# robertteleng/aria-slam

Measured on AMD Instinct MI355X. Metric: frames/s ORB extract+BF-match, 640x480 @2000 kp, higher is better.
Workload: dtype u8

## Files before the change

### aria_slam_amd/csrc/orb_kernels.hip

```cpp
#include <hip/hip_runtime.h>

#include <cfloat>
#include <cstdint>
#include <cstdlib>

#include "common.h"
#include "orb_device.h"
#include "orb_kernels.h"

namespace aria {

struct PatternLaneMajor { uint32_t w[16][16]; };
constexpr PatternLaneMajor make_pattern_lane_major() {
    constexpr int src[1024] = {
#include "orb_pattern_31.inc"
    };
    PatternLaneMajor p{};
    for (int l = 0; l < 16; l++)
        for (int it = 0; it < 16; it++) {
            const int t = 16 * it + l;
            p.w[l][it] = ((uint32_t)(src[4 * t] & 0xFF)) | ((uint32_t)(src[4 * t + 1] & 0xFF) << 8) |
                         ((uint32_t)(src[4 * t + 2] & 0xFF) << 16) | ((uint32_t)(src[4 * t + 3] & 0xFF) << 24);
        }
    return p;
}
__device__ __attribute__((aligned(16))) const PatternLaneMajor kPattern31 = make_pattern_lane_major();

#define ARIA_UMAX_LIST {15, 15, 15, 15, 14, 14, 14, 13, 13, 12, 11, 10, 9, 8, 6, 3}

struct IcMaskLaneMajor { uint32_t m[16][16]; };
constexpr IcMaskLaneMajor make_ic_mask() {
    constexpr int umax[16] = ARIA_UMAX_LIST;
    IcMaskLaneMajor t{};
    for (int l = 0; l < 16; l++)
        for (int k = 0; k < 16; k++) {
            const int r = 2 * k + (l >> 3), j = l & 7;
            uint32_t w = 0;
            for (int b = 0; b < 4 && r < 31; b++) {
                const int u = 4 * j + b - 15, v = r - 15;
                const int au = u < 0 ? -u : u, av = v < 0 ? -v : v;
                if (au <= 15 && au <= umax[av]) w |= 0xFFu << (8 * b);
            }
            t.m[l][k] = w;
        }
    return t;
}
__device__ __attribute__((aligned(16))) const IcMaskLaneMajor kIcMask = make_ic_mask();

typedef short s2v __attribute__((ext_vector_type(2)));
__device__ __forceinline__ void harris_row_pairs(const uint8_t* rowp, int xs, int sh, bool dword_ok, uint32_t* E) {
    uint32_t w0, w1, w2;
    if (dword_ok) {
        const uint32_t* q = reinterpret_cast<const uint32_t*>(rowp + xs);
        w0 = q[0]; w1 = q[1]; w2 = q[2];
    } else {
        const uint8_t* q = rowp + xs;
        w0 = (uint32_t)q[0] | ((uint32_t)q[1] << 8) | ((uint32_t)q[2] << 16) | ((uint32_t)q[3] << 24);
        w1 = (uint32_t)q[4] | ((uint32_t)q[5] << 8) | ((uint32_t)q[6] << 16) | ((uint32_t)q[7] << 24);
        w2 = (uint32_t)q[8] | ((uint32_t)q[9] << 8) | ((uint32_t)q[10] << 16) | ((uint32_t)q[11] << 24);
    }
    const uint32_t a = __builtin_amdgcn_alignbyte(w1, w0, (uint32_t)sh);
    const uint32_t b = __builtin_amdgcn_alignbyte(w2, w1, (uint32_t)sh);
    E[0] = __builtin_amdgcn_perm(0u, a, 0x0c010c00u);
    E[1] = __builtin_amdgcn_perm(0u, a, 0x0c030c02u);
    E[2] = __builtin_amdgcn_perm(0u, b, 0x0c010c00u);
    E[3] = __builtin_amdgcn_perm(0u, b, 0x0c030c02u);
    E[4] = (w2 >> (8 * sh)) & 0xFFu;
}

__device__ __forceinline__ uint32_t pk16_add(uint32_t a, uint32_t b) {
    return __builtin_bit_cast(uint32_t, __builtin_bit_cast(s2v, a) + __builtin_bit_cast(s2v, b));
}
__device__ __forceinline__ uint32_t pk16_sub(uint32_t a, uint32_t b) {
    return __builtin_bit_cast(uint32_t, __builtin_bit_cast(s2v, a) - __builtin_bit_cast(s2v, b));
}

__device__ __forceinline__ float harris_response(const uint8_t* img, int pitch, int x, int y, bool dword_ok) {
    int a = 0, b = 0, c = 0;
    const int xs = (x - 4) & ~3, sh = (x - 4) & 3;
    const uint8_t* base = img + (int64_t)(y - 4) * pitch;
    uint32_t R[9][5];
#pragma unroll
    for (int r = 0; r < 9; r++) harris_row_pairs(base + (int64_t)r * pitch, xs, sh, dword_ok, R[r]);
#pragma unroll
    for (int i = 1; i <= 7; i++) {
        uint32_t sE[5], dE[5];
#pragma unroll
        for (int k = 0; k < 5; k++) {
            sE[k] = pk16_add(pk16_add(R[i - 1][k], R[i + 1][k]), pk16_add(R[i][k], R[i][k]));
            dE[k] = pk16_sub(R[i + 1][k], R[i - 1][k]);
        }
#pragma unroll
        for (int k = 0; k < 4; k++) {
            uint32_t ix = pk16_sub(sE[k + 1], sE[k]);
            const uint32_t dO = __builtin_amdgcn_alignbit(dE[k + 1], dE[k], 16);
            uint32_t iy = pk16_add(pk16_add(dE[k], dE[k + 1]), pk16_add(dO, dO));
            if (k == 3) { ix &= 0xFFFFu; iy &= 0xFFFFu; }
            const s2v vx = __builtin_bit_cast(s2v, ix), vy = __builtin_bit_cast(s2v, iy);
            a = __builtin_amdgcn_sdot2(vx, vx, a, false);
            b = __builtin_amdgcn_sdot2(vy, vy, b, false);
            c = __builtin_amdgcn_sdot2(vx, vy, c, false);
        }
    }
    const float scale = 1.f / ((1 << 2) * 7 * 255.f);
    const float scale_sq_sq = scale * scale * scale * scale;
    const float k = 0.04f;
    return ((float)a * (float)b - (float)c * (float)c - k * ((float)a + (float)b) * ((float)a + (float)b)) * scale_sq_sq;
}

__device__ void select_ovf_item(const Plan& P, const FrameSrc& S, const uint8_t* __restrict__ raw,
                                const uint32_t* __restrict__ cand, const int* __restrict__ cand_cnt,
                                uint4* __restrict__ sel, int* __restrict__ sel_cnt, int* __restrict__ err,
                                int* __restrict__ ovf, unsigned long long* __restrict__ keys, long long keys_cap,
                                uint4* __restrict__ osel, int osel_cap, int frame, int l, int* s_hist, int* s_misc);

template <bool INLINE_OVF, int NT>
__global__ __launch_bounds__(NT) void k_select(Plan P, FrameSrc S, const uint8_t* __restrict__ raw,
                                                const uint32_t* __restrict__ cand, const int* __restrict__ cand_cnt,
                                                uint4* __restrict__ sel, int* __restrict__ sel_cnt,
                                                int* __restrict__ err, unsigned long long* __restrict__ stamps,
                                                int* __restrict__ ovf, int2* __restrict__ ovf_items,
                                                unsigned long long* __restrict__ ovf_keys, long long ovf_keys_cap,
                                                uint4* __restrict__ osel, int osel_cap, int force_bitonic) {
    static_assert(kLevels == 8, "level rotation below assumes 8 levels");
    const int l = (int)((blockIdx.x + blockIdx.y) & 7u), frame = blockIdx.y;
#define SSTAMP(k) do { if (stamps && threadIdx.x == 0) stamps[((size_t)blockIdx.y * kLevels + l) * 8 + (k)] = __builtin_amdgcn_s_memtime(); } while (0)
    SSTAMP(0);
    extern __shared__ __attribute__((aligned(16))) unsigned long long s_keys[];
    __shared__ int s_hist[256];
    __shared__ int s_misc[4];
    __shared__ int s_wsum[NT / 64];
    __shared__ int s_bin[1024];

    const int tid = threadIdx.x;
    const bool lead = tid < 256;
    const LevelGeom g = P.lv[l];
    const uint32_t* clist = cand + (int64_t)frame * P.cand_frame_entries + g.cand_off;
    const int n = min(cand_cnt[frame * kLevels + l], g.cand_cap);
    const int q = g.quota;
    const int kSortCap = P.sort_cap;

    if (q == 0 || n == 0) {
        if (tid == 0) sel_cnt[frame * kLevels + l] = 0;
        return;
    }
    if (lead) s_hist[tid] = 0;
    if (tid == 0) { s_misc[1] = 0; s_misc[2] = 0; }
    __syncthreads();
    constexpr int kUnroll = 8;
    for (int i0 = 0; i0 < n; i0 += NT * kUnroll) {
        uint32_t v[kUnroll];
#pragma unroll
        for (int u = 0; u < kUnroll; u++) {
            const int i = i0 + u * NT + tid;
            v[u] = i < n ? clist[i] : 0u;
        }
#pragma unroll
        for (int u = 0; u < kUnroll; u++)
            if (i0 + u * NT + tid < n) atomicAdd(&s_hist[v[u] >> 22], 1);
    }
    __syncthreads();
    SSTAMP(1);
    {
        const int lane = tid & 63, wv = tid >> 6;
        int c = s_hist[255 - (tid & 255)];
#pragma unroll
        for (int d = 1; d < 64; d <<= 1) {
            const int o = __shfl_up(c, d);
            if (lane >= d) c += o;
        }
        if (lane == 63) s_wsum[wv] = c;
        if (tid == 0) s_misc[0] = 0;
        __syncthreads();
        int before = 0;
#pragma unroll
        for (int w = 0; w < 3; w++)
            if (w < wv) before += s_wsum[w];
        const int cum = c + before;
        const int own = s_hist[255 - (tid & 255)];
        if (lead && n > 2 * q && cum >= 2 * q && cum - own < 2 * q) s_misc[0] = 255 - tid;
        __syncthreads();
    }
    const int thr = s_misc[0];
    for (int i0 = 0; i0 < n; i0 += NT * kUnroll) {
        uint32_t v[kUnroll];
#pragma unroll
        for (int u = 0; u < kUnroll; u++) {
            const int i = i0 + u * NT + tid;
            v[u] = i < n ? clist[i] : 0u;
        }
#pragma unroll
        for (int u = 0; u < kUnroll; u++) {
            const bool keep = i0 + u * NT + tid < n && (int)(v[u] >> 22) >= thr;
            const unsigned long long m = __ballot(keep);
            if (m) {
                const int lane = tid & 63, leader = __ffsll((long long)m) - 1;
                int base = 0;
                if (lane == leader) base = atomicAdd(&s_misc[1], __popcll(m));
                base = __shfl(base, leader);
                const int slot = base + __popcll(m & ((1ull << lane) - 1ull));
                if (keep && slot < kSortCap) s_keys[slot] = (unsigned long long)v[u];
            }
        }
    }
    __syncthreads();
    SSTAMP(2);
    int pitch;
    const uint8_t* img = raw_level_ptr(P, S, raw, frame, l, pitch);
    {
        const int ns = min(s_misc[1], kSortCap);
        for (int i = tid; i < ns; i += NT) {
            const uint32_t cd = (uint32_t)s_keys[i];
            const int x = cd & 0x7FF, y = (cd >> 11) & 0x7FF;
            const float r = harris_response(img, pitch, x, y, (l > 0) || S.aligned4);
            uint32_t u = __float_as_uint(r);
            u = (u & 0x80000000u) ? ~u : (u | 0x80000000u);
            s_keys[i] = ((unsigned long long)(~u) << 32) | ((uint32_t)y << 16) | (uint32_t)x;
        }
    }
    __syncthreads();
    SSTAMP(3);
    int n1 = s_misc[1];
    if (n1 > kSortCap) {
        if (INLINE_OVF) {
            __shared__ __attribute__((aligned(8))) int s_ovm[8];
            if (!lead) return;
            select_ovf_item(P, S, raw, cand, cand_cnt, sel, sel_cnt, err, ovf, ovf_keys, ovf_keys_cap, osel, osel_cap, frame, l,
                            s_hist, s_ovm);
            return;
        }
        if (tid == 0) {
            sel_cnt[frame * kLevels + l] = 0;
            const int it = atomicAdd(&ovf[0], 1);
            if (it < kOvfItems) ovf_items[it] = make_int2(frame, l);
            else atomicOr(err, ERRBIT_SORT_OVERFLOW);
        }
        return;
    }
    __shared__ int s_srt[2];
    auto hbin = [](unsigned long long kk) { return (int)min((uint32_t)(kk >> 53), 1023u); };
    const bool cut = n1 > q + 64;
    for (int i = tid; i < 1024; i += NT) s_bin[i] = 0;
    if (tid == 0) { s_srt[0] = 1023; s_srt[1] = 0; }
    __syncthreads();
    for (int i = tid; i < n1; i += NT) atomicAdd(&s_bin[hbin(s_keys[i])], 1);
    __syncthreads();
    {
        const int lane = tid & 63, wv = tid >> 6;
        int b[4], tot = 0;
#pragma unroll
        for (int k = 0; k < 4; k++) { b[k] = lead ? s_bin[4 * tid + k] : 0; tot += b[k]; }
        int c = tot;
#pragma unroll
        for (int d = 1; d < 64; d <<= 1) {
            const int o = __shfl_up(c, d);
            if (lane >= d) c += o;
        }
        if (lane == 63) s_wsum[wv] = c;
        if (tid == 0) s_misc[1] = 0;
        __syncthreads();
        int run = c - tot;
#pragma unroll
        for (int w = 0; w < 3; w++)
            if (w < wv) run += s_wsum[w];
#pragma unroll
        for (int k = 0; k < 4; k++) {
            if (lead) s_bin[4 * tid + k] = run;
            if (lead && cut && run < q && run + b[k] >= q) s_srt[0] = 4 * tid + k;
            run += b[k];
        }
        __syncthreads();
        const int bc = s_srt[0];
        int mx = 0;
#pragma unroll
        for (int k = 0; k < 4; k++)
            if (lead && 4 * tid + k <= bc) mx = max(mx, b[k]);
        if (mx > 0) atomicMax(&s_srt[1], mx);
    }
    const int bcut = s_srt[0];
    if (cut) {
        for (int i0 = 0; i0 < n1; i0 += NT) {
            const int i = i0 + tid;
            const unsigned long long kk = i < n1 ? s_keys[i] : ~0ull;
            const bool keep = i < n1 && hbin(kk) <= bcut;
            __syncthreads();
            const unsigned long long m = __ballot(keep);
            if (m) {
                const int lane = tid & 63, leader = __ffsll((long long)m) - 1;
                int base = 0;
                if (lane == leader) base = atomicAdd(&s_misc[1], __popcll(m));
                base = __shfl(base, leader);
                if (keep) s_keys[base + __popcll(m & ((1ull << lane) - 1ull))] = kk;
            }
        }
        __syncthreads();
        n1 = s_misc[1];
    } else {
        __syncthreads();
    }
    const int upper = kSortCap >> 1;
    if (n1 <= upper && s_srt[1] <= 512 && !force_bitonic) {
        unsigned long long* s_up = s_keys + upper;
        for (int i = tid; i < n1; i += NT) {
            const unsigned long long kk = s_keys[i];
            s_up[atomicAdd(&s_bin[hbin(kk)], 1)] = kk;
        }
        __syncthreads();
        for (int i = tid; i < n1; i += NT) {
            const unsigned long long kk = s_up[i];
            const int b = hbin(kk);
            const int lo = b ? s_bin[b - 1] : 0, hi = s_bin[b];
            int r = lo;
            for (int j0 = lo; j0 < hi; j0 += 8) {
                unsigned long long o[8];
#pragma unroll
                for (int u = 0; u < 8; u++) o[u] = s_up[min(j0 + u, hi - 1)];
#pragma unroll
                for (int u = 0; u < 8; u++) r += (j0 + u < hi && o[u] < kk) ? 1 : 0;
            }
            s_keys[r] = kk;
        }
    } else {
        int np = 1;
        while (np < n1) np <<= 1;
        for (int i = n1 + tid; i < np; i += NT) s_keys[i] = ~0ull;
        __syncthreads();
        auto steps_of = [](int kk) { int n = 0; for (int jj = kk >> 1; jj > 0; jj >>= 1) n++; return n; };
        for (int k = 2; k <= np; k <<= 1) {
            int j = k >> 1;
            if (steps_of(k) & 1) {
                __syncthreads();
// ... 43 lines not shown
            __shared__ __attribute__((aligned(8))) int s_ovm[8];
            if (!lead) return;
            select_ovf_item(P, S, raw, cand, cand_cnt, sel, sel_cnt, err, ovf, ovf_keys, ovf_keys_cap, osel, osel_cap, frame, l,
                            s_hist, s_ovm);
            return;
        }
        if (tid == 0) {
            sel_cnt[frame * kLevels + l] = 0;
            const int it = atomicAdd(&ovf[0], 1);
            if (it < kOvfItems) ovf_items[it] = make_int2(frame, l);
            else atomicOr(err, ERRBIT_SEL_OVERFLOW);
        }
        return;
    }
    uint4* out = sel + (int64_t)frame * P.sel_frame_entries + g.sel_off;
    const int ts = (((g.w + 31) >> 5) * ((g.h + 31) >> 5) <= 1024) ? 5 : 6;
    const int tiles_x = (g.w + (1 << ts) - 1) >> ts, n_bins = tiles_x * ((g.h + (1 << ts) - 1) >> ts);
    for (int i = tid; i < n_bins; i += NT) s_bin[i] = 0;
    __syncthreads();
    for (int i = tid; i < n2; i += NT) {
        const uint32_t xy = (uint32_t)s_keys[i];
        atomicAdd(&s_bin[((xy >> (16 + ts)) * tiles_x) + ((xy & 0xFFFFu) >> ts)], 1);
    }
    __syncthreads();
    {
        const int lane = tid & 63, wv = tid >> 6;
        int b[4], tot = 0;
#pragma unroll
        for (int k = 0; k < 4; k++) { b[k] = (lead && 4 * tid + k < n_bins) ? s_bin[4 * tid + k] : 0; tot += b[k]; }
        int c = tot;
#pragma unroll
        for (int d = 1; d < 64; d <<= 1) {
            const int o = __shfl_up(c, d);
            if (lane >= d) c += o;
        }
        __syncthreads();
        if (lane == 63) s_wsum[wv] = c;
        __syncthreads();
        int run = c - tot;
#pragma unroll
        for (int w = 0; w < 3; w++)
            if (w < wv) run += s_wsum[w];
#pragma unroll
        for (int k = 0; k < 4; k++) {
            if (lead && 4 * tid + k < n_bins) s_bin[4 * tid + k] = run;
            run += b[k];
        }
    }
    __syncthreads();
    for (int i = tid; i < n2; i += NT) {
        const unsigned long long kk = s_keys[i];
        uint32_t u = ~(uint32_t)(kk >> 32);
        u = (u & 0x80000000u) ? (u & 0x7FFFFFFFu) : ~u;
        const uint32_t xy = (uint32_t)kk;
        const int pos = atomicAdd(&s_bin[((xy >> (16 + ts)) * tiles_x) + ((xy & 0xFFFFu) >> ts)], 1);
        out[pos] = make_uint4(xy, u, (uint32_t)i, 0u);
    }
    if (tid == 0) sel_cnt[frame * kLevels + l] = n2;
    SSTAMP(5);
#undef SSTAMP
}

__device__ __forceinline__ unsigned long long ovf_ld(const unsigned long long* p) {
    return __hip_atomic_load(p, __ATOMIC_RELAXED, __HIP_MEMORY_SCOPE_AGENT);
}
__device__ __forceinline__ void ovf_st(unsigned long long* p, unsigned long long v) {
    __hip_atomic_store(p, v, __ATOMIC_RELAXED, __HIP_MEMORY_SCOPE_AGENT);
}

__device__ __attribute__((noinline)) void select_ovf_item(const Plan& P, const FrameSrc& S, const uint8_t* __restrict__ raw,
                                const uint32_t* __restrict__ cand, const int* __restrict__ cand_cnt,
                                uint4* __restrict__ sel, int* __restrict__ sel_cnt, int* __restrict__ err,
                                int* __restrict__ ovf, unsigned long long* __restrict__ keys, long long keys_cap,
                                uint4* __restrict__ osel, int osel_cap, int frame, int l, int* s_hist, int* s_misc) {
    const int tid = threadIdx.x;
    {
        const LevelGeom g = P.lv[l];
        const uint32_t* clist = cand + (int64_t)frame * P.cand_frame_entries + g.cand_off;
        const int n = min(cand_cnt[frame * kLevels + l], g.cand_cap);
        const int q = g.quota;
        __syncthreads();
        s_hist[tid] = 0;
        if (tid < 8) s_misc[tid] = 0;
        __syncthreads();
        for (int i = tid; i < n; i += 256) atomicAdd(&s_hist[clist[i] >> 22], 1);
        __syncthreads();
        if (tid == 0) {
            int thr = 0, n1 = n;
            if (n > 2 * q) {
                int cum = 0;
                for (int sc = 255; sc >= 0; sc--) {
                    cum += s_hist[sc];
                    if (cum >= 2 * q) { thr = sc; n1 = cum; break; }
                }
            }
            long long np = 1;
            while (np < n1) np <<= 1;
            const long long base = (long long)atomicAdd(reinterpret_cast<unsigned long long*>(ovf + 2), (unsigned long long)np);
            s_misc[0] = thr;
            if (base + np > keys_cap) { atomicOr(err, ERRBIT_SORT_OVERFLOW); s_misc[3] = -1; }
            else { s_misc[3] = 0; }
            reinterpret_cast<long long*>(s_misc + 6)[0] = base;
            s_misc[5] = n1;
        }
        __syncthreads();
        if (s_misc[3] < 0) { if (tid == 0) sel_cnt[frame * kLevels + l] = 0; return; }
        const int thr = s_misc[0], n1 = s_misc[5];
        unsigned long long* K = keys + reinterpret_cast<long long*>(s_misc + 6)[0];
        long long np = 1;
        while (np < n1) np <<= 1;
        int pitch;
        const uint8_t* img = raw_level_ptr(P, S, raw, frame, l, pitch);
        for (int i0 = 0; i0 < n; i0 += 256) {
            const int i = i0 + tid;
            const uint32_t cd = i < n ? clist[i] : 0u;
            const bool keep = i < n && (int)(cd >> 22) >= thr;
            unsigned long long key = 0;
            if (keep) {
                const int x = cd & 0x7FF, y = (cd >> 11) & 0x7FF;
                const float r = harris_response(img, pitch, x, y, (l > 0) || S.aligned4);
                uint32_t u = __float_as_uint(r);
                u = (u & 0x80000000u) ? ~u : (u | 0x80000000u);
                key = ((unsigned long long)(~u) << 32) | ((uint32_t)y << 16) | (uint32_t)x;
            }
            const unsigned long long m = __ballot(keep);
            if (m) {
                const int lane = tid & 63, leader = __ffsll((long long)m) - 1;
                int base = 0;
                if (lane == leader) base = atomicAdd(&s_misc[1], __popcll(m));
                base = __shfl(base, leader);
                if (keep) ovf_st(&K[base + __popcll(m & ((1ull << lane) - 1ull))], key);
            }
        }
        for (long long i = n1 + tid; i < np; i += 256) ovf_st(&K[i], ~0ull);
        __syncthreads();
        for (long long k = 2; k <= np; k <<= 1)
            for (long long j = k >> 1; j > 0; j >>= 1) {
                for (long long t = tid; t < (np >> 1); t += 256) {
                    const long long a = ((t & ~(j - 1)) << 1) | (t & (j - 1)), b = a | j;
                    const unsigned long long xa = ovf_ld(&K[a]), xb = ovf_ld(&K[b]);
                    if ((xa > xb) == ((a & k) == 0)) { ovf_st(&K[a], xb); ovf_st(&K[b], xa); }
                }
                __syncthreads();
            }
        int n2 = n1;
        if (n1 > q) {
            const uint32_t cut = (uint32_t)(ovf_ld(&K[q - 1]) >> 32);
            for (int i = q + tid; i < n1; i += 256)
                if ((uint32_t)(ovf_ld(&K[i]) >> 32) == cut) atomicAdd(&s_misc[2], 1);
            __syncthreads();
            n2 = q + s_misc[2];
        }
        const int extra = max(n2 - g.sel_cap, 0), extra4 = (extra + 3) & ~3;
        if (tid == 0) {
            int ob = 0;
            if (extra4 > 0) {
                ob = atomicAdd(&ovf[1], extra4);
                if (ob + extra4 > osel_cap) { atomicOr(err, ERRBIT_SEL_OVERFLOW); ob = -1; }
            }
            s_misc[4] = ob;
        }
        __syncthreads();
        const int ob = s_misc[4];
        if (ob < 0) n2 = g.sel_cap;
        uint4* out = sel + (int64_t)frame * P.sel_frame_entries + g.sel_off;
        const uint32_t tag = (uint32_t)frame | ((uint32_t)l << 24);
        for (int i = tid; i < n2; i += 256) {
            const unsigned long long kk = ovf_ld(&K[i]);
            uint32_t u = ~(uint32_t)(kk >> 32);
            u = (u & 0x80000000u) ? (u & 0x7FFFFFFFu) : ~u;
            const uint4 rec = make_uint4((uint32_t)kk, u, (uint32_t)i, tag);
            if (i < g.sel_cap) out[i] = rec;
            else osel[ob + (i - g.sel_cap)] = rec;
        }
        if (ob >= 0)
            for (int i = extra + tid; i < extra4; i += 256) osel[ob + i] = make_uint4(0u, 0u, 0xFFFFFFFFu, tag);
        if (tid == 0) sel_cnt[frame * kLevels + l] = n2;
    }
}

__global__ __launch_bounds__(256) void k_select_ovf(Plan P, FrameSrc S, const uint8_t* __restrict__ raw,
                                                    const uint32_t* __restrict__ cand, const int* __restrict__ cand_cnt,
                                                    uint4* __restrict__ sel, int* __restrict__ sel_cnt, int* __restrict__ err,
                                                    int* __restrict__ ovf, const int2* __restrict__ ovf_items,
                                                    unsigned long long* __restrict__ keys, long long keys_cap,
                                                    uint4* __restrict__ osel, int osel_cap) {
    __shared__ int s_hist[256];
    __shared__ __attribute__((aligned(8))) int s_misc[8];
    const int n_items = min(ovf[0], kOvfItems);
    for (int it = blockIdx.x; it < n_items; it += gridDim.x)
        select_ovf_item(P, S, raw, cand, cand_cnt, sel, sel_cnt, err, ovf, keys, keys_cap, osel, osel_cap, ovf_items[it].x,
                        ovf_items[it].y, s_hist, s_misc);
}

__device__ __forceinline__ float fast_atan2_deg(float y, float x) {
    const float p1 = 0.9997878412794807f * (float)(180 / 3.1415926535897932384626433832795);
    const float p3 = -0.3258083974640975f * (float)(180 / 3.1415926535897932384626433832795);
    const float p5 = 0.1555786518463281f * (float)(180 / 3.1415926535897932384626433832795);
    const float p7 = -0.04432655554792128f * (float)(180 / 3.1415926535897932384626433832795);
    const float ax = fabsf(x), ay = fabsf(y);
    float a, c, c2;
    if (ax >= ay) {
        c = ay / (ax + (float)DBL_EPSILON);
        c2 = c * c;
        a = (((p7 * c2 + p5) * c2 + p3) * c2 + p1) * c;
    } else {
        c = ax / (ay + (float)DBL_EPSILON);
        c2 = c * c;
        a = 90.f - (((p7 * c2 + p5) * c2 + p3) * c2 + p1) * c;
    }
    if (x < 0) a = 180.f - a;
    if (y < 0) a = 360.f - a;
    return a;
}

__device__ __forceinline__ void det_sincos(double x, double& s, double& c) {
    const double invpio2 = 6.36619772367581382433e-01;
    const double pio2_hi = 1.57079632673412561417e+00;
    const double pio2_lo = 6.07710050650619224932e-11;
    const double S1 = -1.66666666666666324348e-01, S2 = 8.33333333332248946124e-03,
                 S3 = -1.98412698298579493134e-04, S4 = 2.75573137070700676789e-06,
                 S5 = -2.50507602534068634195e-08, S6 = 1.58969099521155010221e-10;
    const double C1 = 4.16666666666666019037e-02, C2 = -1.38888888888741095749e-03,
                 C3 = 2.48015872894767294178e-05, C4 = -2.75573143513906633035e-07,
                 C5 = 2.08757232129817482790e-09, C6 = -1.13596475577881948265e-11;
    const double fn = floor(x * invpio2 + 0.5);
    const double r = (x - fn * pio2_hi) - fn * pio2_lo;
    const double z = r * r;
    const double sp = S2 + z * (S3 + z * (S4 + z * (S5 + z * S6)));
    const double sn = r + (z * r) * (S1 + z * sp);
    const double cp = z * (C1 + z * (C2 + z * (C3 + z * (C4 + z * (C5 + z * C6)))));
    const double cs = 1.0 - (0.5 * z - z * cp);
    const int qd = (int)fn & 3;
    s = (qd == 0) ? sn : (qd == 1) ? cs : (qd == 2) ? -sn : -cs;
    c = (qd == 0) ? cs : (qd == 1) ? -sn : (qd == 2) ? -cs : sn;
}

__device__ __forceinline__ int wave_sum(int v) {
    v += __builtin_amdgcn_update_dpp(0, v, 0xB1, 0xF, 0xF, true);
    v += __builtin_amdgcn_update_dpp(0, v, 0x4E, 0xF, 0xF, true);
    v += __builtin_amdgcn_update_dpp(0, v, 0x141, 0xF, 0xF, true);
    v += __builtin_amdgcn_update_dpp(0, v, 0x140, 0xF, 0xF, true);
    v += __builtin_amdgcn_update_dpp(0, v, 0x142, 0xA, 0xF, false);
    v += __builtin_amdgcn_update_dpp(0, v, 0x143, 0xC, 0xF, false);
    return __builtin_amdgcn_readlane(v, 63);
}

constexpr int kDescR = 18;
constexpr int kDescRows = 2 * kDescR + 1;
constexpr int kDescPitch = 64;
constexpr int kDescWaves = 2;
constexpr int kDescKp = 4 * kDescWaves;
constexpr int kIcPitch = 48;
struct __attribute__((packed, aligned(4))) DwordQuad { uint32_t a, b, c, d; };

__device__ __forceinline__ int row8_sum(int v) {
    v += __builtin_amdgcn_update_dpp(0, v, 0xB1, 0xF, 0xF, true);
    v += __builtin_amdgcn_update_dpp(0, v, 0x4E, 0xF, 0xF, true);
    v += __builtin_amdgcn_update_dpp(0, v, 0x141, 0xF, 0xF, true);
    return v;
}

__device__ __forceinline__ int row16_sum(int v) {
    v += __builtin_amdgcn_update_dpp(0, v, 0xB1, 0xF, 0xF, true);
    v += __builtin_amdgcn_update_dpp(0, v, 0x4E, 0xF, 0xF, true);
    v += __builtin_amdgcn_update_dpp(0, v, 0x141, 0xF, 0xF, true);
    v += __builtin_amdgcn_update_dpp(0, v, 0x140, 0xF, 0xF, true);
    return v;
}

constexpr int kDescArenaBlocks = 32;
constexpr int kDescQ = 10;
constexpr int kDescPitchQ = 4 * kDescQ;

constexpr int kDesc16Kp = 16;
__device__ __forceinline__ int row_src(int r) { return (((int)(threadIdx.x & 0x30)) | r) << 2; }
__device__ __forceinline__ int row_pick(int v, int src) { return __builtin_amdgcn_ds_bpermute(src, v); }

__host__ __device__ __forceinline__ int desc16_waves_per_frame(const Plan& P) {
    int w = 0;
    for (int i = 0; i < kLevels; i++) w += (P.lv[i].sel_cap + kDesc16Kp - 1) / kDesc16Kp;
    return w;
}

template <int MODE>
__device__ __forceinline__ void describe16(const Plan& P, const FrameSrc& S, const uint8_t* __restrict__ raw,
                                           const uint8_t* __restrict__ blur, const uint4* __restrict__ sel,
                                           const int* __restrict__ sel_cnt, aria_keypoint* __restrict__ kps,
                                           uint8_t* __restrict__ desc, int* __restrict__ counts, int kp_cap,
                                           int* __restrict__ err, int n_frames, int blocks_per_frame,
                                           unsigned long long* __restrict__ stamps,
                                           const uint4* __restrict__ osel, const int* __restrict__ ovf, int osel_cap,
                                           const int blk_in) {
    constexpr bool ARENA = MODE == 1;
#define DSTAMP16(k) do { if (stamps && (threadIdx.x & 63) == 0) stamps[((size_t)blockIdx.x * kDescWaves + (threadIdx.x >> 6)) * 8 + (k)] = __builtin_amdgcn_s_memtime(); } while (0)
    DSTAMP16(0);
    constexpr int kPatchBytes = kDescPitchQ * kDescPitchQ;
    static_assert(kPatchBytes >= 31 * kIcPitch && kPatchBytes % 16 == 0, "the raw window shares the allocation");
    __shared__ __attribute__((aligned(16))) uint8_t s_patch[kDescKp][kPatchBytes];
    const int lane = threadIdx.x & 63, wv = threadIdx.x >> 6;
    const int grp = lane >> 4, l16 = lane & 15;
    const int rs = l16 & 3;
    uint8_t* const win = s_patch[wv * 4 + grp];

    int frame = 0, l = 0, base = 0;
    uint4 sv;
    bool valid;
    uint32_t act = 0;
    if constexpr (!ARENA) {
        const int blk = __builtin_amdgcn_readfirstlane(blk_in);
        const int xcd = blk & 7, j = blk >> 3;
        frame = __builtin_amdgcn_readfirstlane((j / blocks_per_frame) * 8 + xcd);
        if (frame >= n_frames) return;
        const int w = __builtin_amdgcn_readfirstlane((j % blocks_per_frame) * kDescWaves + wv);
        const int* cnt = sel_cnt + frame * kLevels;
        int total = 0, wl = 0, i0 = -1;
#pragma unroll
        for (int i = 0; i < kLevels; i++) {
            const int ci = cnt[i];
            const int nw = (P.lv[i].sel_cap + kDesc16Kp - 1) / kDesc16Kp;
            if (w >= wl && w < wl + nw) { l = i; base = total; i0 = kDesc16Kp * (w - wl); }
            wl += nw;
            total += ci;
        }
        if (w == 0 && lane == 0) {
            counts[frame] = min(total, kp_cap);
            if (total > kp_cap) atomicMax(err + 2, total);
        }
        if (i0 < 0) return;
        l = __builtin_amdgcn_readfirstlane(l);
        base = __builtin_amdgcn_readfirstlane(base);
        const int nk = min(kDesc16Kp, min(cnt[l], P.lv[l].sel_cap) - i0);
        if (nk <= 0) return;
        act = (1u << ((nk + 3) >> 2)) - 1u;
        const int k = 4 * rs + grp;
        valid = l16 < 4 && k < nk;
        sv = sel[(int64_t)frame * P.sel_frame_entries + P.lv[l].sel_off + i0 + min(k, nk - 1)];
    } else {
        const int e0 = __builtin_amdgcn_readfirstlane((blk_in * kDescWaves + wv) * kDesc16Kp);
        const int n_arena = min(ovf[1], osel_cap);
        if (e0 >= n_arena) return;
        const bool blk_ok = e0 + 4 * rs < n_arena;
        const int eb = e0 + 4 * rs;
        const bool live = blk_ok && osel[eb + grp].z != 0xFFFFFFFFu;
        const unsigned long long vm = __ballot(live && l16 < 4);
        const int nkr = __popcll(vm & (0x0001000100010001ull << rs));
        valid = l16 < 4 && grp < nkr;
#pragma unroll
        for (int r = 0; r < 4; r++)
            if ((vm & (0x0001000100010001ull << r)) && act == (1u << r) - 1u) act |= 1u << r;
        if (act == 0) return;
        sv = blk_ok ? osel[eb + min(grp, max(nkr, 1) - 1)] : make_uint4(0u, 0u, 0u, 0u);
    }
    auto round_fl = [&](int r, int& fr, int& lr) {
        if constexpr (ARENA) {
            const uint32_t tag = (uint32_t)__builtin_amdgcn_readlane((int)sv.w, r);
            fr = (int)(tag & 0xFFFFFFu);
            lr = (int)(tag >> 24);
        } else {
            fr = frame; lr = l;
        }
    };
    const int x_s = sv.x & 0xFFFF, y_s = sv.x >> 16;
    if (stamps) { asm volatile("s_waitcnt vmcnt(0)" ::: "memory"); }
    DSTAMP16(1);

    uint32_t icm[16];
#pragma unroll
    for (int k = 0; k < 16; k += 4) {
        const uint4 m4 = *reinterpret_cast<const uint4*>(&kIcMask.m[l16][k]);
        icm[k] = m4.x; icm[k + 1] = m4.y; icm[k + 2] = m4.z; icm[k + 3] = m4.w;
    }
    const int rr = l16 / 3, cc = l16 - 3 * rr;
    const int hp = l16 >> 3, jj = l16 & 7;
    const uint32_t wu = 0x04030201u + 0x04040404u * (uint32_t)jj;
    DwordQuad rv[7];
    int sh_n = 0;
    auto raw_issue = [&](int r) {
        int fr, lr;
        round_fl(r, fr, lr);
        int pitch;
        const uint8_t* img = raw_level_ptr(P, S, raw, fr, lr, pitch);
        const bool raw_dword = __builtin_amdgcn_readfirstlane((lr > 0) || S.aligned4) != 0;
        const bool raw_a16 = __builtin_amdgcn_readfirstlane((lr > 0) || S.aligned16) != 0;
        const int xy = row_pick((int)sv.x, row_src(r));
        const int x = xy & 0xFFFF, y = (int)((uint32_t)xy >> 16);
        const int xr = raw_a16 ? ((x - kHalfPatch) & ~15) : ((x - kHalfPatch) & ~3);
        sh_n = (x - xr) - kHalfPatch;
        const uint32_t o = (uint32_t)((y - kHalfPatch) * pitch + xr + 16 * cc);
        if (raw_dword) {
#pragma unroll
            for (int k = 0; k < 7; k++) {
                const int row = (5 * k + 5 < 31) ? 5 * k + rr : min(5 * k + rr, 30);
                rv[k] = *reinterpret_cast<const DwordQuad*>(img + (o + (uint32_t)(row * pitch)));
            }
        } else {
#pragma unroll
            for (int k = 0; k < 7; k++) {
                const int row = (5 * k + 5 < 31) ? 5 * k + rr : min(5 * k + rr, 30);
                const uint8_t* q = img + (o + (uint32_t)(row * pitch));
                rv[k].a = (uint32_t)q[0] | ((uint32_t)q[1] << 8) | ((uint32_t)q[2] << 16) | ((uint32_t)q[3] << 24);
                rv[k].b = (uint32_t)q[4] | ((uint32_t)q[5] << 8) | ((uint32_t)q[6] << 16) | ((uint32_t)q[7] << 24);
                rv[k].c = (uint32_t)q[8] | ((uint32_t)q[9] << 8) | ((uint32_t)q[10] << 16) | ((uint32_t)q[11] << 24);
                rv[k].d = (uint32_t)q[12] | ((uint32_t)q[13] << 8) | ((uint32_t)q[14] << 16) | ((uint32_t)q[15] << 24);
            }
        }
    };
    constexpr int kPv = 7;
    DwordQuad pv[kPv];
    int pq[kPv], pc[kPv];
#pragma unroll
    for (int k = 0; k < kPv; k++) {
        const int p = min(16 * k + l16, kDescQ * kDescQ - 1);
        pq[k] = (p * 205) >> 11;
        pc[k] = p - kDescQ * pq[k];
    }
    auto blur_issue = [&](int r) {
        int fr, lr;
        round_fl(r, fr, lr);
        const uint8_t* bl = blur + (int64_t)fr * P.blur_frame_bytes + P.lv[lr].blur_off;
        const int qp = P.lv[lr].pitch * 4;
        const int xy = row_pick((int)sv.x, row_src(r));
        const int x = xy & 0xFFFF, y = (int)((uint32_t)xy >> 16);
        const uint32_t o = (uint32_t)(((y - kDescR) >> 2) * qp + ((x - kDescR) >> 2) * 16);
#pragma unroll
        for (int k = 0; k < kPv; k++)
            pv[k] = *reinterpret_cast<const DwordQuad*>(bl + (o + (uint32_t)(pq[k] * qp + pc[k] * 16)));
    };

    int m10_s = 0, m01_s = 0;
    const int nr = 32 - __builtin_clz(act);
    auto moment_round = [&](int r, auto next) {
        const int sh = sh_n;
        {
            uint8_t* sr = win + 16 * cc;
#pragma unroll
            for (int k = 0; k < 7; k++) {
                const int row = (5 * k + 5 < 31) ? 5 * k + rr : min(5 * k + rr, 30);
                *reinterpret_cast<uint4*>(sr + row * kIcPitch) = make_uint4(rv[k].a, rv[k].b, rv[k].c, rv[k].d);
            }
        }
        next();
        __builtin_amdgcn_wave_barrier();
        const uint8_t* rbase = win + 4 * jj + (sh & ~3);
        uint32_t acc_u = 0, acc_v = 0, acc_s = 0;
#pragma unroll
        for (int k = 0; k < 16; k++) {
            const int rw = min(2 * k + hp, 30);
            const uint32_t lo = *reinterpret_cast<const uint32_t*>(rbase + rw * kIcPitch);
            const uint32_t hi = *reinterpret_cast<const uint32_t*>(rbase + rw * kIcPitch + 4);
            const uint32_t pix = __builtin_amdgcn_alignbyte(hi, lo, sh) & icm[k];
            acc_u = __builtin_amdgcn_udot4(pix, wu, acc_u, false);
            acc_v = __builtin_amdgcn_udot4(pix, 0x01010101u * (uint32_t)(2 * k + 1), acc_v, false);
            acc_s = __builtin_amdgcn_sad_u8(pix, 0u, acc_s);
        }
        const int sum_u = row16_sum((int)acc_u), sum_v = row16_sum((int)acc_v);
        const int s_half = row8_sum((int)acc_s);
        const int s_othr = __builtin_amdgcn_update_dpp(0, s_half, 0x140, 0xF, 0xF, true);
        const int s_all = s_half + s_othr;
        const int s_hp1 = hp ? s_half : s_othr;
        if (l16 == r) {
            m10_s = sum_u - 16 * s_all;
            m01_s = sum_v + s_hp1 - 16 * s_all;
        }
        __builtin_amdgcn_wave_barrier();
    };
    raw_issue(0);
#pragma unroll 1
    for (int r = 0; r < nr - 1; r++) moment_round(r, [&] { raw_issue(r + 1); });
    moment_round(nr - 1, [&] { blur_issue(0); });
    if (stamps) { asm volatile("s_waitcnt vmcnt(0) lgkmcnt(0)" ::: "memory"); }
    DSTAMP16(2);

    const float angle_s = fast_atan2_deg((float)m01_s, (float)m10_s);
    float ang = angle_s;
    ang *= (float)(3.1415926535897932384626433832795 / 180.f);
    double sd, cd;
    det_sincos((double)ang, sd, cd);
    const float a_s = (float)cd, b_s = (float)sd;
    int base_s = base, frame_s = frame, l_s = l;
    if constexpr (ARENA) {
        const uint32_t tag = sv.w;
        frame_s = (int)(tag & 0xFFFFFFu);
        l_s = (int)(tag >> 24);
        base_s = 0;
        if (valid) {
            const int* cnt = sel_cnt + frame_s * kLevels;
            for (int i = 0; i < l_s; i++) base_s += cnt[i];
        }
    }
    const int oidx_s = base_s + (int)sv.z;
    const bool fits_s = oidx_s < kp_cap;
    if (valid && !fits_s) atomicOr(err, ERRBIT_KPCAP);
    const int orow_s = (valid && fits_s) ? oidx_s : -1;
    if (stamps) { asm volatile("s_waitcnt vmcnt(0) lgkmcnt(0)" ::: "memory"); }
    DSTAMP16(3);

    int pat[16];
#pragma unroll
    for (int it = 0; it < 16; it += 4) {
        const uint4 p4 = *reinterpret_cast<const uint4*>(&kPattern31.w[l16][it]);
        pat[it] = (int)p4.x; pat[it + 1] = (int)p4.y; pat[it + 2] = (int)p4.z; pat[it + 3] = (int)p4.w;
    }
    typedef float f2 __attribute__((ext_vector_type(2)));
    const f2 magic = {12582912.0f, 12582912.0f};
    constexpr uint32_t kMagicBits = 0x4B400000u;
    constexpr int kPitchL = kDescPitchQ;
#pragma unroll 1
    for (int r = 0; r < nr; r++) {
        const int src = row_src(r);
        const int xy = row_pick((int)sv.x, src);
        const int x = xy & 0xFFFF, y = (int)((uint32_t)xy >> 16);
        const int xs = (x - kDescR) & ~3, ys = (y - kDescR) & ~3;
        const float a = __int_as_float(row_pick(__float_as_int(a_s), src));
        const float b = __int_as_float(row_pick(__float_as_int(b_s), src));
        const int orow = row_pick(orow_s, src);
        __builtin_amdgcn_wave_barrier();
#pragma unroll
        for (int k = 0; k < kPv; k++) {
            uint32_t* d = reinterpret_cast<uint32_t*>(win + (4 * pq[k]) * kPitchL + 4 * pc[k]);
            d[0] = pv[k].a; d[kPitchL / 4] = pv[k].b; d[2 * kPitchL / 4] = pv[k].c; d[3 * kPitchL / 4] = pv[k].d;
        }
        if (r + 1 < nr) blur_issue(r + 1);
        const uint8_t* bc = win + (y - ys) * kPitchL + (x - xs);
        __builtin_amdgcn_wave_barrier();
        const f2 aa = {a, a}, bb = {b, b}, nbb = {-b, -b};
        const uint8_t* bc0 = bc - (size_t)(0x400000u * (uint32_t)kPitchL + kMagicBits);
#pragma unroll
        for (int it = 0; it < 16; it++) asm volatile("" : "+v"(pat[it]));
        uint32_t mine = 0;
#pragma unroll
        for (int it = 0; it < 16; it++) {
            const float px0 = (float)(signed char)(pat[it] & 0xFF), py0 = (float)(signed char)((pat[it] >> 8) & 0xFF);
            const float px1 = (float)(signed char)((pat[it] >> 16) & 0xFF), py1 = (float)(signed char)((pat[it] >> 24) & 0xFF);
            const f2 PX = {px0, px1}, PY = {py0, py1};
            const f2 fx = PX * aa + PY * nbb + magic;
            const f2 fy = PX * bb + PY * aa + magic;
            const uint32_t o0 = __umul24(__float_as_uint(fy.x), kPitchL) + __float_as_uint(fx.x);
            const uint32_t o1 = __umul24(__float_as_uint(fy.y), kPitchL) + __float_as_uint(fx.y);
            const int t0 = bc0[o0];
            const int t1 = bc0[o1];
            const unsigned long long m = __ballot(t0 < t1);
            if (__builtin_amdgcn_inverse_ballot_w64(0x0001000100010001ull << it)) mine = (uint32_t)(m >> (16 * grp)) & 0xFFFFu;
        }
        if (orow >= 0) {
            int fr, lr;
            round_fl(r, fr, lr);
            *reinterpret_cast<uint16_t*>(desc + ((int64_t)fr * kp_cap + orow) * 32 + 2 * l16) = (uint16_t)mine;
        }
        __builtin_amdgcn_wave_barrier();
    }
    if (stamps) { asm volatile("s_waitcnt vmcnt(0) lgkmcnt(0)" ::: "memory"); }
    DSTAMP16(4);

    if (orow_s >= 0) {
        float scale = P.lv[l].scale;
        if constexpr (ARENA) {
#pragma unroll
            for (int i = 1; i < kLevels; i++)
                if (l_s == i) scale = P.lv[i].scale;
        }
        aria_keypoint k;
        k.x = (float)x_s * scale;
        k.y = (float)y_s * scale;
        k.size = kPatchSize * scale;
        k.angle = angle_s;
        k.response = __uint_as_float(sv.y);
        k.octave = l_s;
        kps[(int64_t)frame_s * kp_cap + orow_s] = k;
    }
    DSTAMP16(5);
#undef DSTAMP16
}

template <int MODE, bool Q4, bool W16 = false>
__global__ __launch_bounds__(64 * kDescWaves, W16 && MODE == 0 ? 4 : 1) void k_describe(Plan P, FrameSrc S, const uint8_t* __restrict__ raw,
                                                  const uint8_t* __restrict__ blur, const uint4* __restrict__ sel,
                                                  const int* __restrict__ sel_cnt, aria_keypoint* __restrict__ kps,
                                                  uint8_t* __restrict__ desc, int* __restrict__ counts, int kp_cap,
                                                  int* __restrict__ err, int n_frames, int blocks_per_frame,
                                                  unsigned long long* __restrict__ stamps,
                                                  const uint4* __restrict__ osel, const int* __restrict__ ovf, int osel_cap) {
    if constexpr (W16) {
        static_assert(Q4 && MODE < 2, "the 16-keypoint form is the batch Q4 form");
        if constexpr (MODE == 0) {
            describe16<0>(P, S, raw, blur, sel, sel_cnt, kps, desc, counts, kp_cap, err, n_frames, blocks_per_frame, stamps,
                          osel, ovf, osel_cap, (int)blockIdx.x);
        } else {
            const int n_blk = (min(ovf[1], osel_cap) + kDescWaves * kDesc16Kp - 1) / (kDescWaves * kDesc16Kp);
            for (int blk = blockIdx.x; blk < n_blk; blk += gridDim.x)
                describe16<1>(P, S, raw, blur, sel, sel_cnt, kps, desc, counts, kp_cap, err, n_frames, blocks_per_frame,
                              stamps, osel, ovf, osel_cap, blk);
        }
        return;
    }
#define DSTAMP(k) do { if (stamps && (threadIdx.x & 63) == 0) stamps[((size_t)blockIdx.x * kDescWaves + (threadIdx.x >> 6)) * 8 + (k)] = __builtin_amdgcn_s_memtime(); } while (0)
    DSTAMP(0);
    constexpr int kPatchBytes = Q4 ? kDescPitchQ * kDescPitchQ : kDescRows * kDescPitch;
    static_assert(kPatchBytes >= 31 * kIcPitch && kPatchBytes % 16 == 0, "the raw window shares the allocation");
    __shared__ __attribute__((aligned(16))) uint8_t s_patch[kDescKp][kPatchBytes];
    uint8_t (*s_raw)[kPatchBytes] = s_patch;
    const int lane = threadIdx.x & 63, wv = threadIdx.x >> 6;
    const int grp = lane >> 4, l16 = lane & 15;
    const int n_regular = MODE == 2 ? (int)gridDim.x - kDescArenaBlocks : (int)gridDim.x;
    auto describe_block = [&](const int blk_in, const bool ARENA) {
    const int blk = __builtin_amdgcn_readfirstlane(blk_in);
    int frame, l = 0, base = 0, nk;
    uint4 sv;
    if (!ARENA) {
        const int xcd = blk & 7, j = blk >> 3;
        frame = __builtin_amdgcn_readfirstlane((j / blocks_per_frame) * 8 + xcd);
        if (frame >= n_frames) return;
        const int jm = __builtin_amdgcn_readfirstlane(j % blocks_per_frame);
        const int slot0 = __builtin_amdgcn_readfirstlane(jm * kDescKp + wv * 4);
        const int* cnt = sel_cnt + frame * kLevels;
        int total = 0;
#pragma unroll
        for (int i = 0; i < kLevels; i++) {
            const int ci = cnt[i];
            if (i > 0 && slot0 >= P.lv[i].sel_off) { l = i; base = total; }
            total += ci;
        }
        if (slot0 == 0 && lane == 0) {
            counts[frame] = min(total, kp_cap);
            if (total > kp_cap) atomicMax(err + 2, total);
        }
        if (slot0 >= P.sel_frame_entries) return;
        l = __builtin_amdgcn_readfirstlane(l);
        base = __builtin_amdgcn_readfirstlane(base);
        const int i0 = slot0 - P.lv[l].sel_off;
        nk = min(4, min(cnt[l], P.lv[l].sel_cap) - i0);
        if (nk <= 0) return;
        sv = sel[(int64_t)frame * P.sel_frame_entries + slot0 + min(grp, nk - 1)];
    } else {
        const int e0 = blk * kDescKp + wv * 4;
        if (e0 >= min(ovf[1], osel_cap)) return;
        const uint4 mine = osel[e0 + grp];
        const unsigned long long vm = __ballot(mine.z != 0xFFFFFFFFu && l16 == 0);
        nk = __popcll(vm);
        if (nk <= 0) return;
        const uint32_t tag = (uint32_t)__builtin_amdgcn_readfirstlane((int)mine.w);
        frame = (int)(tag & 0xFFFFFFu);
        l = (int)(tag >> 24);
        const int* cnt = sel_cnt + frame * kLevels;
        for (int i = 0; i < l; i++) base += cnt[i];
        sv = osel[e0 + min(grp, nk - 1)];
    }
    const LevelGeom g = P.lv[l];
    const bool valid = grp < nk;
    const int oidx = base + (int)sv.z;
    const bool fits = oidx < kp_cap;
    if (valid && !fits && l16 == 0) atomicOr(err, ERRBIT_KPCAP);
    const int x = sv.x & 0xFFFF, y = sv.x >> 16;
    if (stamps) { asm volatile("s_waitcnt vmcnt(0)" ::: "memory"); }
    DSTAMP(1);

    uint32_t icm[16];
#pragma unroll
    for (int k = 0; k < 16; k += 4) {
        const uint4 m4 = *reinterpret_cast<const uint4*>(&kIcMask.m[l16][k]);
        icm[k] = m4.x; icm[k + 1] = m4.y; icm[k + 2] = m4.z; icm[k + 3] = m4.w;
    }
    int pat[16];
#pragma unroll
    for (int it = 0; it < 16; it += 4) {
        const uint4 p4 = *reinterpret_cast<const uint4*>(&kPattern31.w[l16][it]);
        pat[it] = (int)p4.x; pat[it + 1] = (int)p4.y; pat[it + 2] = (int)p4.z; pat[it + 3] = (int)p4.w;
    }

    const uint8_t* bl = blur + (int64_t)frame * P.blur_frame_bytes + g.blur_off;
    const int xs = Q4 ? ((x - kDescR) & ~3) : ((x - kDescR) & ~15);
    const int ys = Q4 ? ((y - kDescR) & ~3) : (y - kDescR);
    constexpr int kPv = Q4 ? 7 : 10;
    DwordQuad pv[kPv];
    int pq[kPv], pc[kPv];
    if constexpr (Q4) {
        const int64_t qp = (int64_t)g.pitch * 4;
        const uint8_t* gp = bl + (int64_t)(ys >> 2) * qp + (xs >> 2) * 16;
#pragma unroll
        for (int k = 0; k < kPv; k++) {
            const int p = min(16 * k + l16, kDescQ * kDescQ - 1);
            pq[k] = (p * 205) >> 11;
            pc[k] = p - kDescQ * pq[k];
            pv[k] = *reinterpret_cast<const DwordQuad*>(gp + pq[k] * qp + pc[k] * 16);
        }
    } else {
        const int r4 = l16 >> 2, c4 = l16 & 3;
        const int64_t p64 = g.pitch;
        const uint8_t* gp = bl + (int64_t)(y - kDescR) * p64 + xs + 16 * c4;
#pragma unroll
        for (int k = 0; k < 10; k++) {
            const int row = (4 * k + 4 <= kDescRows) ? 4 * k + r4 : min(4 * k + r4, kDescRows - 1);
            pv[k] = *reinterpret_cast<const DwordQuad*>(gp + row * p64);
        }
        (void)pq; (void)pc;
    }
    const int rr = l16 / 3, cc = l16 - 3 * rr;
    int pitch;
    const uint8_t* img = raw_level_ptr(P, S, raw, frame, l, pitch);
    const bool raw_dword = __builtin_amdgcn_readfirstlane((l > 0) || S.aligned4) != 0;
    const bool raw_a16 = __builtin_amdgcn_readfirstlane((l > 0) || S.aligned16) != 0;
    const int xr = raw_a16 ? ((x - kHalfPatch) & ~15) : ((x - kHalfPatch) & ~3);
    {
        uint8_t* sr = s_raw[wv * 4 + grp] + 16 * cc;
        const int64_t p64 = pitch;
        const uint8_t* gp = img + (int64_t)(y - kHalfPatch) * p64 + xr + 16 * cc;
        DwordQuad rv[7];
        if (raw_dword) {
#pragma unroll
            for (int k = 0; k < 7; k++) {
                const int row = (5 * k + 5 < 31) ? 5 * k + rr : min(5 * k + rr, 30);
                rv[k] = *reinterpret_cast<const DwordQuad*>(gp + row * p64);
            }
        } else {
#pragma unroll
            for (int k = 0; k < 7; k++) {
                const int row = (5 * k + 5 < 31) ? 5 * k + rr : min(5 * k + rr, 30);
                const uint8_t* q = gp + row * p64;
                rv[k].a = (uint32_t)q[0] | ((uint32_t)q[1] << 8) | ((uint32_t)q[2] << 16) | ((uint32_t)q[3] << 24);
                rv[k].b = (uint32_t)q[4] | ((uint32_t)q[5] << 8) | ((uint32_t)q[6] << 16) | ((uint32_t)q[7] << 24);
                rv[k].c = (uint32_t)q[8] | ((uint32_t)q[9] << 8) | ((uint32_t)q[10] << 16) | ((uint32_t)q[11] << 24);
                rv[k].d = (uint32_t)q[12] | ((uint32_t)q[13] << 8) | ((uint32_t)q[14] << 16) | ((uint32_t)q[15] << 24);
            }
        }
#pragma unroll
        for (int k = 0; k < 7; k++) {
            const int row = (5 * k + 5 < 31) ? 5 * k + rr : min(5 * k + rr, 30);
            *reinterpret_cast<uint4*>(sr + row * kIcPitch) = make_uint4(rv[k].a, rv[k].b, rv[k].c, rv[k].d);
        }
    }
    if (stamps) { asm volatile("s_waitcnt vmcnt(0) lgkmcnt(0)" ::: "memory"); }
    DSTAMP(2);
    __builtin_amdgcn_wave_barrier();

    const int sh = (x - xr) - kHalfPatch;
    const int hp = l16 >> 3, jj = l16 & 7;
    const uint8_t* rbase = s_raw[wv * 4 + grp] + 4 * jj + (sh & ~3);
    const uint32_t wu = 0x04030201u + 0x04040404u * (uint32_t)jj;
    uint32_t acc_u = 0, acc_v = 0, acc_s = 0;
#pragma unroll
    for (int k = 0; k < 16; k++) {
        const int r = min(2 * k + hp, 30);
        const uint32_t lo = *reinterpret_cast<const uint32_t*>(rbase + r * kIcPitch);
        const uint32_t hi = *reinterpret_cast<const uint32_t*>(rbase + r * kIcPitch + 4);
        const uint32_t pix = __builtin_amdgcn_alignbyte(hi, lo, sh) & icm[k];
        acc_u = __builtin_amdgcn_udot4(pix, wu, acc_u, false);
        acc_v = __builtin_amdgcn_udot4(pix, 0x01010101u * (uint32_t)(2 * k + 1), acc_v, false);
        acc_s = __builtin_amdgcn_sad_u8(pix, 0u, acc_s);
    }
    const int sum_u = row16_sum((int)acc_u), sum_v = row16_sum((int)acc_v);
    const int s_half = row8_sum((int)acc_s);
    const int s_othr = __builtin_amdgcn_update_dpp(0, s_half, 0x140, 0xF, 0xF, true);
    const int s_all = s_half + s_othr;
    const int s_hp1 = hp ? s_half : s_othr;
    const int m10 = sum_u - 16 * s_all;
    const int m01 = sum_v + s_hp1 - 16 * s_all;
    const float angle = fast_atan2_deg((float)m01, (float)m10);
    DSTAMP(3);

    float ang = angle;
    ang *= (float)(3.1415926535897932384626433832795 / 180.f);
    double sd, cd;
    det_sincos((double)ang, sd, cd);
    const float a = (float)cd, b = (float)sd;
    __builtin_amdgcn_wave_barrier();
    constexpr int kPitchL = Q4 ? kDescPitchQ : kDescPitch;
    if constexpr (Q4) {
        uint8_t* sp = s_patch[wv * 4 + grp];
#pragma unroll
        for (int k = 0; k < kPv; k++) {
            uint32_t* d = reinterpret_cast<uint32_t*>(sp + (4 * pq[k]) * kPitchL + 4 * pc[k]);
            d[0] = pv[k].a; d[kPitchL / 4] = pv[k].b; d[2 * kPitchL / 4] = pv[k].c; d[3 * kPitchL / 4] = pv[k].d;
        }
// ... 316 lines not shown
```

Measured before the change: 394,100.

## Compute intensity-centroid moments with i8 MFMA instead of LDS dot4 rounds

For the non-arena descriptor path, the orientation moments (m10, m01) are now computed as a matrix product. Raw patch rows are loaded straight from global memory, shifted into alignment with alignbyte, and recentred to signed bytes by XOR 0x80. They are then multiplied against a constexpr int8 weight table of masked u and v coordinates using mfma_i32_16x16x64_i8. This replaces the per-keypoint LDS window staging and the udot4/sad accumulation rounds. The gain depends on zero-sum weights, which static asserts enforce. The trade-off is more register pressure from the 8 in-flight pieces, a ds_bpermute per step, and extra LDS for the weight table.

```diff
diff --git a/aria_slam_amd/csrc/ic_moment_weights.h b/aria_slam_amd/csrc/ic_moment_weights.h
--- /dev/null
+++ b/aria_slam_amd/csrc/ic_moment_weights.h
@@ -0,0 +1,60 @@
+#pragma once
+#include <cstdint>
+
+namespace aria {
+
+#define ARIA_UMAX_LIST {15, 15, 15, 15, 14, 14, 14, 13, 13, 12, 11, 10, 9, 8, 6, 3}
+
+constexpr int kIcPieces = 64;
+constexpr int kIcPieceBytes = 16;
+
+struct IcMomentWeights { int8_t w[2][kIcPieces][kIcPieceBytes]; };
+
+constexpr IcMomentWeights make_ic_moment_weights() {
+    constexpr int umax[16] = ARIA_UMAX_LIST;
+    IcMomentWeights t{};
+    for (int p = 0; p < kIcPieces; p++)
+        for (int j = 0; j < kIcPieceBytes; j++) {
+            const int row = p >> 1, half = p & 1;
+            const int u = 16 * half + j - 15, v = row - 15;
+            const int au = u < 0 ? -u : u, av = v < 0 ? -v : v;
+            const bool in = row < 31 && au <= 15 && au <= umax[av];
+            t.w[0][p][j] = (int8_t)(in ? u : 0);
+            t.w[1][p][j] = (int8_t)(in ? v : 0);
+        }
+    return t;
+}
+
+constexpr int ic_moment_weight_sum(int role) {
+    const IcMomentWeights t = make_ic_moment_weights();
+    int s = 0;
+    for (int p = 0; p < kIcPieces; p++)
+        for (int j = 0; j < kIcPieceBytes; j++) s += t.w[role][p][j];
+    return s;
+}
+constexpr long long ic_moment_weight_abs_sum(int role) {
+    const IcMomentWeights t = make_ic_moment_weights();
+    long long s = 0;
+    for (int p = 0; p < kIcPieces; p++)
+        for (int j = 0; j < kIcPieceBytes; j++) s += t.w[role][p][j] < 0 ? -t.w[role][p][j] : t.w[role][p][j];
+    return s;
+}
+constexpr int kIcTailStepLo = 4, kIcTailStepHi = 10;
+constexpr bool ic_moment_tail_is_zero_outside(int lo, int hi) {
+    const IcMomentWeights t = make_ic_moment_weights();
+    for (int p = 0; p < kIcPieces; p++) {
+        const int step = p >> 2;
+        if ((p & 1) == 0 || (step >= lo && step <= hi)) continue;
+        for (int role = 0; role < 2; role++)
+            for (int j = 13; j < kIcPieceBytes; j++)
+                if (t.w[role][p][j] != 0) return false;
+    }
+    return true;
+}
+static_assert(ic_moment_tail_is_zero_outside(kIcTailStepLo, kIcTailStepHi), "a step outside the range needs its fifth dword");
+static_assert(ic_moment_weight_sum(0) == 0 && ic_moment_weight_sum(1) == 0,
+              "the moments of I - 128 equal the moments of I only while each role's weights sum to 0");
+static_assert(128 * ic_moment_weight_abs_sum(0) < (1ll << 31) && 128 * ic_moment_weight_abs_sum(1) < (1ll << 31),
+              "the int32 accumulator holds every moment");
+
+}
diff --git a/aria_slam_amd/csrc/orb_kernels.hip b/aria_slam_amd/csrc/orb_kernels.hip
--- a/aria_slam_amd/csrc/orb_kernels.hip
+++ b/aria_slam_amd/csrc/orb_kernels.hip
@@ -5,6 +5,7 @@
 #include <cstdlib>
 
 #include "common.h"
+#include "ic_moment_weights.h"
 #include "orb_device.h"
 #include "orb_kernels.h"
 
@@ -26,7 +27,11 @@
 }
 __device__ __attribute__((aligned(16))) const PatternLaneMajor kPattern31 = make_pattern_lane_major();
 
-#define ARIA_UMAX_LIST {15, 15, 15, 15, 14, 14, 14, 13, 13, 12, 11, 10, 9, 8, 6, 3}
+
+#ifndef ARIA_DESC_MOMENTS_LDS
+#define ARIA_DESC_MOMENTS_LDS 0
+#endif
+__device__ __attribute__((aligned(16))) const IcMomentWeights kIcMomentW = make_ic_moment_weights();
 
 struct IcMaskLaneMajor { uint32_t m[16][16]; };
 constexpr IcMaskLaneMajor make_ic_mask() {
@@ -676,16 +681,28 @@
     const int grp = lane >> 4, l16 = lane & 15;
     const int rs = l16 & 3;
     uint8_t* const win = s_patch[wv * 4 + grp];
+#if ARIA_DESC_MOMENTS_LDS
+    constexpr bool MOM_MFMA = false;
+#else
+    constexpr bool MOM_MFMA = !ARENA;
+#endif
+    static_assert(sizeof(IcMomentWeights) == 2 * 16 * 64, "two 16-byte pieces of the weight table per lane");
+    __shared__ __attribute__((aligned(16))) int8_t s_icw[kDescWaves][sizeof(IcMomentWeights)];
 
     int frame = 0, l = 0, base = 0;
     uint4 sv;
     bool valid;
     uint32_t act = 0;
+    uint4 wq0 = make_uint4(0u, 0u, 0u, 0u), wq1 = wq0;
     if constexpr (!ARENA) {
         const int blk = __builtin_amdgcn_readfirstlane(blk_in);
         const int xcd = blk & 7, j = blk >> 3;
         frame = __builtin_amdgcn_readfirstlane((j / blocks_per_frame) * 8 + xcd);
         if (frame >= n_frames) return;
+        if constexpr (MOM_MFMA) {
+            wq0 = reinterpret_cast<const uint4*>(&kIcMomentW.w[0][0][0])[lane];
+            wq1 = reinterpret_cast<const uint4*>(&kIcMomentW.w[1][0][0])[lane];
+        }
         const int w = __builtin_amdgcn_readfirstlane((j % blocks_per_frame) * kDescWaves + wv);
         const int* cnt = sel_cnt + frame * kLevels;
         int total = 0, wl = 0, i0 = -1;
@@ -739,6 +756,84 @@
     if (stamps) { asm volatile("s_waitcnt vmcnt(0)" ::: "memory"); }
     DSTAMP16(1);
 
+    constexpr int kPv = 7;
+    DwordQuad pv[kPv];
+    int pq[kPv], pc[kPv];
+#pragma unroll
+    for (int k = 0; k < kPv; k++) {
+        const int p = min(16 * k + l16, kDescQ * kDescQ - 1);
+        pq[k] = (p * 205) >> 11;
+        pc[k] = p - kDescQ * pq[k];
+    }
+    auto blur_issue = [&](int r) {
+        int fr, lr;
+        round_fl(r, fr, lr);
+        const uint8_t* bl = blur + (int64_t)fr * P.blur_frame_bytes + P.lv[lr].blur_off;
+        const int qp = P.lv[lr].pitch * 4;
+        const int xy = row_pick((int)sv.x, row_src(r));
+        const int x = xy & 0xFFFF, y = (int)((uint32_t)xy >> 16);
+        const uint32_t o = (uint32_t)(((y - kDescR) >> 2) * qp + ((x - kDescR) >> 2) * 16);
+#pragma unroll
+        for (int k = 0; k < kPv; k++)
+            pv[k] = *reinterpret_cast<const DwordQuad*>(bl + (o + (uint32_t)(pq[k] * qp + pc[k] * 16)));
+    };
+
+    int m10_s = 0, m01_s = 0;
+    const int nr = 32 - __builtin_clz(act);
+    if constexpr (MOM_MFMA) {
+    typedef int v4i __attribute__((ext_vector_type(4)));
+    typedef v4i __attribute__((aligned(1))) v4i_unaligned;
+    typedef uint32_t __attribute__((aligned(1))) u32_unaligned;
+    int pitch;
+    const uint8_t* img = raw_level_ptr(P, S, raw, frame, l, pitch);
+    const bool exact = __builtin_amdgcn_readfirstlane((l == 0) && !S.aligned4) != 0;
+    const int xy = row_pick((int)sv.x, ((l16 >> 2) * 16 + (l16 & 3)) << 2);
+    const int x = xy & 0xFFFF, y = (int)((uint32_t)xy >> 16);
+    const int prow = grp >> 1, phalf = grp & 1;
+    const uint32_t sh = exact ? 0u : (uint32_t)(x - kHalfPatch) & 3u;
+    const uint32_t o = (uint32_t)((y - kHalfPatch + prow) * pitch + (x - kHalfPatch) + 16 * phalf) - sh;
+    struct Piece { v4i q; uint32_t e; };
+    auto piece = [&](int k) -> Piece {
+        const uint32_t off = k < 15 ? o + (uint32_t)(2 * k * pitch) : o + (uint32_t)((30 - prow) * pitch);
+        Piece t;
+        t.q = *reinterpret_cast<const v4i_unaligned*>(img + off);
+        t.e = 0u;
+        if (k >= kIcTailStepLo && k <= kIcTailStepHi) t.e = *reinterpret_cast<const u32_unaligned*>(img + off + 16);
+        return t;
+    };
+    const int up16 = ((lane + 16) & 63) << 2;
+    auto operand = [&](const Piece& t, int k) -> v4i {
+        v4i r;
+        uint32_t e = (uint32_t)__builtin_amdgcn_ds_bpermute(up16, t.q[0]);
+        if (k >= kIcTailStepLo && k <= kIcTailStepHi) e = phalf ? t.e : e;
+        r[0] = (int)__builtin_amdgcn_alignbyte((uint32_t)t.q[1], (uint32_t)t.q[0], sh);
+        r[1] = (int)__builtin_amdgcn_alignbyte((uint32_t)t.q[2], (uint32_t)t.q[1], sh);
+        r[2] = (int)__builtin_amdgcn_alignbyte((uint32_t)t.q[3], (uint32_t)t.q[2], sh);
+        r[3] = (int)__builtin_amdgcn_alignbyte(e, (uint32_t)t.q[3], sh);
+        return r ^ (int)0x80808080;
+    };
+    const int8_t* wb = s_icw[wv] + ((l16 >> 2) & 1) * (kIcPieces * kIcPieceBytes) + grp * kIcPieceBytes;
+    Piece a[8];
+#pragma unroll
+    for (int k = 0; k < 8; k++) a[k] = piece(k);
+    reinterpret_cast<uint4*>(s_icw[wv])[lane] = wq0;
+    reinterpret_cast<uint4*>(s_icw[wv])[64 + lane] = wq1;
+    __builtin_amdgcn_wave_barrier();
+    v4i acc0 = {0, 0, 0, 0}, acc1 = {0, 0, 0, 0};
+#pragma unroll
+    for (int k = 0; k < 16; k++) {
+        if (k == 8) blur_issue(0);
+        const v4i av = operand(a[k & 7], k);
+        const v4i bv = *reinterpret_cast<const v4i*>(wb + 4 * kIcPieceBytes * k);
+        if (k & 1) acc1 = __builtin_amdgcn_mfma_i32_16x16x64_i8(av, bv, acc1, 0, 0, 0);
+        else acc0 = __builtin_amdgcn_mfma_i32_16x16x64_i8(av, bv, acc0, 0, 0, 0);
+        if (k < 8) a[k] = piece(k + 8);
+    }
+    const v4i acc = acc0 + acc1;
+    const int sel = (l16 & 2) ? ((l16 & 1) ? acc[3] : acc[2]) : ((l16 & 1) ? acc[1] : acc[0]);
+    m10_s = sel;
+    m01_s = __builtin_amdgcn_update_dpp(0, sel, 0x104, 0xF, 0xF, true);
+    } else {
     uint32_t icm[16];
 #pragma unroll
     for (int k = 0; k < 16; k += 4) {
@@ -780,30 +875,6 @@
             }
         }
     };
-    constexpr int kPv = 7;
-    DwordQuad pv[kPv];
-    int pq[kPv], pc[kPv];
-#pragma unroll
-    for (int k = 0; k < kPv; k++) {
-        const int p = min(16 * k + l16, kDescQ * kDescQ - 1);
-        pq[k] = (p * 205) >> 11;
-        pc[k] = p - kDescQ * pq[k];
-    }
-    auto blur_issue = [&](int r) {
-        int fr, lr;
-        round_fl(r, fr, lr);
-        const uint8_t* bl = blur + (int64_t)fr * P.blur_frame_bytes + P.lv[lr].blur_off;
-        const int qp = P.lv[lr].pitch * 4;
-        const int xy = row_pick((int)sv.x, row_src(r));
-        const int x = xy & 0xFFFF, y = (int)((uint32_t)xy >> 16);
-        const uint32_t o = (uint32_t)(((y - kDescR) >> 2) * qp + ((x - kDescR) >> 2) * 16);
-#pragma unroll
-        for (int k = 0; k < kPv; k++)
-            pv[k] = *reinterpret_cast<const DwordQuad*>(bl + (o + (uint32_t)(pq[k] * qp + pc[k] * 16)));
-    };
-
-    int m10_s = 0, m01_s = 0;
-    const int nr = 32 - __builtin_clz(act);
     auto moment_round = [&](int r, auto next) {
         const int sh = sh_n;
         {
@@ -843,6 +914,7 @@
 #pragma unroll 1
     for (int r = 0; r < nr - 1; r++) moment_round(r, [&] { raw_issue(r + 1); });
     moment_round(nr - 1, [&] { blur_issue(0); });
+    }
     if (stamps) { asm volatile("s_waitcnt vmcnt(0) lgkmcnt(0)" ::: "memory"); }
     DSTAMP16(2);
 
```

Result: faster. 403,100, median of 6 (+2.3%).
